# BindsNET/bindsnet

Measured on AMD Instinct MI355X. Metric: simulated timesteps/sec (whole node), DiehlAndCook2015 784->400 batch32, higher is better.
Workload: dtype f32

## Files before the change

### bindsnet_amd/_lib.py

```python
import ctypes as C
import os

_HERE = os.path.dirname(os.path.abspath(__file__))
LIB_PATH = os.path.join(_HERE, "lib", "libsnnhip.so")
if os.environ.get("SNN_DEVELOPER") == "1" and os.environ.get("SNN_LIB_OVERRIDE"):
    import warnings
    LIB_PATH = os.environ["SNN_LIB_OVERRIDE"]
    warnings.warn(f"bindsnet_amd: SNN_LIB_OVERRIDE is active, loading {LIB_PATH} instead of the in-tree library", RuntimeWarning)

SNN_OK, SNN_ERR_NOISE, SNN_ERR_TIMEOUT, SNN_ERR_RETRY = 0, -4, -6, -7
ABI_VERSION = 8


_EPOCH = [0]


def epoch() -> int:
    return _EPOCH[0]


def touch() -> None:
    _EPOCH[0] += 1


# ... 111 lines not shown
    "snn_dc_arbitrate": ([_vp, _vp, _i, _i, C.POINTER(DcParams), _vp, _ll, _vp, _vp, _vp, _vp], _i),
    "snn_stdp_postpre": ([_vp] * 5 + [_i, _i, _i, _f, _f, _i, _f, _f, _i, _f, _i, _f, _i, _vp], _i),
    "snn_conv2d_postpre": ([_vp] * 5 + [_i] * 9 + [_f, _f, _f, _i, _f, _i, _f, _vp, _vp], _i),
    "snn_stdp_hebbian": ([_vp] * 5 + [_i, _i, _i, _f, _f, _i, _f, _i, _f, _i, _f, _vp], _i),
    "snn_conv2d_mstdp_step": ([_vp] * 6 + [_i] * 8 + [_f] * 7 + [_i, _f, _i, _f, _vp], _i),
    "snn_mstdpet_step": ([_vp] * 8 + [_i, _i] + [_f] * 10 + [_i, _f, _i, _f, _vp], _i),
    "snn_mstdp_step": ([_vp] * 7 + [_i, _i, _i, _f, _vp, _f, _f, _f, _f, _f, _f, _i, _f, _i, _f, _vp], _i),
    "snn_normalize": ([_vp, _i, _i, _f, _i, _vp, _vp], _i),
    "snn_normalize_conv2d": ([_vp, _i, _i, _f, _vp], _i),
    "snn_rng_fill_exponential": ([_vp, _vp, _i, _i, _vp, _vp, _vp], _i),
    "snn_encode_bernoulli": ([_vp, _vp, _i, _i, _f, _vp, _vp], _i),
    "snn_encode_poisson": ([_vp, _i, _i, _f, C.c_ulonglong, _vp, _vp], _i),
    "snn_fill_segments": ([C.POINTER(FillSegment), _i, _vp], _i),
    "snn_dist_unique_id": ([_vp], _i),
    "snn_dist_init": ([_i, _i, _vp, C.POINTER(_vp)], _i),
    "snn_dist_world": ([_vp, C.POINTER(_i), C.POINTER(_i)], _i),
    "snn_dist_allreduce_dw": ([_vp, _vp, _ll, _vp], _i),
    "snn_dist_allgather_step": ([_vp, _vp, _vp, _ll, _vp], _i),
    "snn_dist_destroy": ([_vp], _i),
    "snn_net_run": ([C.POINTER(LayerDesc), _i, C.POINTER(ConnDesc), _i, C.POINTER(RunDesc), _vp], _i),
    "snn_net_workspace_bytes": ([C.POINTER(LayerDesc), _i, C.POINTER(ConnDesc), _i, C.POINTER(RunDesc)], C.c_ulonglong),
    "snn_plan_name": ([], C.c_char_p),
    "snn_dc2015_last_form": ([], C.c_int),
    "snn_set_plan_mode": ([_i], None),
    "snn_graph_stats": ([C.POINTER(C.c_int)] * 3, None),
    "snn_profile_enable": ([_i], None),
    "snn_profile_collect": ([C.POINTER(C.c_double), C.POINTER(C.c_int)], _i),
}


def exported_symbols():
    return sorted(_SIGS)


def lib():
    global _lib
    if _lib is None:
        if not os.path.exists(LIB_PATH):
            raise SnnError(f"{LIB_PATH} is missing: build it with `make -C bindsnet_amd/csrc` "
                           "(python __graft_entry__.py build). There is no fallback path.")
        L = C.CDLL(LIB_PATH)
        for name, (args, res) in _SIGS.items():
            fn = getattr(L, name)
            fn.argtypes, fn.restype = args, res
        if L.snn_abi_version() != ABI_VERSION:
            raise SnnError(f"libsnnhip ABI {L.snn_abi_version()} != binding {ABI_VERSION}")
# ... 33 lines not shown
        try:
            for _ in range(max(1, repeats)):
                net.run(dict(inputs), time=time)
                net.reset_state_variables()
                if not net.last_plan.startswith("dc2015-resident"):
                    break
            net.sync()
            torch.cuda.synchronize()
            s, n = C.c_double(0), C.c_int(0)
            check(L.snn_profile_collect(C.byref(s), C.byref(n)), "profile_collect")
        finally:
            L.snn_profile_enable(0)
    if n.value == 0:
        return None
    plan = net.last_plan
    if plan.startswith("dc2015-resident"):
        form = L.snn_dc2015_last_form()
        return {"kernel": resident_kernel_name(form) + " (one launch per network.run())", "resident_form": form, "avg_ms": s.value / n.value, "n": n.value,
                "timesteps_per_launch": int(round(time / net.dt))}
    kernel = "k_dc2015_step (one launch per timestep)" if plan != "generic" else "generic plan: all launches of one timestep"
    return {"kernel": kernel, "avg_ms": s.value / n.value, "n": n.value, "timesteps_per_launch": 1}


def graph_stats():
    a, b, c = C.c_int(0), C.c_int(0), C.c_int(0)
    lib().snn_graph_stats(C.byref(a), C.byref(b), C.byref(c))
    return a.value, b.value, c.value
```

### bindsnet_amd/csrc/snn_dc2015.hip

```cpp
#include <string.h>
#include <stdio.h>
#include <stdlib.h>
#include <vector>
#include <algorithm>
#include "snn_dc2015.hpp"

unsigned long long snn_twolayer_workspace_bytes(const snn_layer_desc *L, int nL, const snn_conn_desc *C, int nC,
                                                const snn_run_desc *R);
bool snn_prof_begin(int t, hipStream_t st);
bool snn_prof_active();
void snn_prof_end(hipStream_t st);

namespace {

template <class SUM, bool FULL>
__device__ __forceinline__ void stdp_rows(const DcCtx &c, int nact, const uint16_t *arows, const uint32_t *rowmask,
                                          const uint32_t *colmask, const uint8_t *__restrict__ sbytes,
                                          const float *xnu0, const float *__restrict__ xsrc, float *wtile, int c0, int tid,
                                          int Emain, const float *pre_w) {
    const int B = c.B, Nin = c.Nin, N = c.N;
    const int nitems = nact * CW;
    const int q = tid % CW;
    for (int base = 0; base < nitems; base += NT * 8) {
        float wv[8]; int ev[8]; int iv[8];
// ... 501 lines not shown
}

size_t lds_bytes(int B, int Nin, int N) {
    const int NW = (N + 31) / 32;
    auto al = [](size_t x) { return (x + 15) & ~(size_t)15; };
    return al((size_t)digest_lds_words(B, Nin) * 4) + 3 * al((size_t)B * NW * 4) +
           (size_t)MAXB * CW * 4 + 8 * 624 * 4 + NCAND * 4 + MAXB * 8 + 2 * MAXB * LR * 2 + 2 * MAXB * 4 + 2 * 32 * 4 + 32 +
           (size_t)Nin * CW * 4 + 2 * MAXB * CW * 4;
}


}

static size_t fused_workspace(int B, int Nin, int N) {
    const int NW = (N + 31) / 32;
    auto al = [](size_t x) { return (x + 255) & ~(size_t)255; };
    return 4 * al((size_t)B * NW * 4) + al((size_t)B * Nin * 4) + al(sizeof(snn_rng_state));
}

static thread_local int g_last_form = -1;
static thread_local unsigned long long g_ws_key_in = 0;
void snn_dc2015_ws_key_in(unsigned long long key) { g_ws_key_in = key; }
constexpr int kAsyncDefault = 1;
static size_t resident_summary_bytes(int N) { return (size_t)4 * ((N + 1) / 2) * 4 * 8; }
static size_t resident_gran_bytes(int B, int N) { return (size_t)4 * ((N + 1) / 2) * ((B + 1) / 2) * 8; }
constexpr size_t kAsyncCtlBytes = 8 * 11 * 8 + 16 * 4 + 64;

static size_t resident_second_bytes(int B, int N) {
    auto al = [](size_t x) { return (x + 255) & ~(size_t)255; };
    return al(resident_gran_bytes(B, N)) + al(resident_summary_bytes(N));
}
static size_t resident_extra(int B, int Nin, int N, int T) {
    auto al = [](size_t x) { return (x + 255) & ~(size_t)255; };
    return al(resident_gran_bytes(B, N)) + al(resident_summary_bytes(N)) + al(kAsyncCtlBytes) + al((size_t)(T + 1 + 16) * 4) + al((size_t)(T + 1) * B * Nin * 4) +
           2 * resident_second_bytes(B, N);
}

constexpr size_t kResidentMaxExtra = (size_t)2 << 30;

static size_t fused_workspace_total(int B, int Nin, int N, int T) {
    auto al = [](size_t x) { return (x + 255) & ~(size_t)255; };
    const size_t extra = resident_extra(B, Nin, N, T);
    return fused_workspace(B, Nin, N) + al((size_t)(T + 1) * digest_words(B, Nin) * 4) + (extra <= kResidentMaxExtra ? extra : 0);
}

static bool matches(const snn_layer_desc *L, int nL, const snn_conn_desc *C, int nC, const snn_run_desc *R) {
    if (nL != 3 || nC != 3) return false;
    if (L[0].kind != SNN_LAYER_INPUT || L[1].kind != SNN_LAYER_DC || L[2].kind != SNN_LAYER_LIF) return false;
    if (L[1].n != L[2].n) return false;
    for (int k = 0; k < 3; ++k) if (C[k].kind != SNN_CONN_MCC || C[k].bias) return false;
    if (C[0].src != 0 || C[0].dst != 1 || C[1].src != 1 || C[1].dst != 2 || C[2].src != 2 || C[2].dst != 1) return false;
    if (C[1].rule != SNN_RULE_NONE || C[2].rule != SNN_RULE_NONE) return false;
    if (C[0].rule != SNN_RULE_NONE && C[0].rule != SNN_RULE_POSTPRE) return false;
    if (C[0].rule == SNN_RULE_POSTPRE && (C[0].wdecay != 1.0f || !L[0].x || !L[1].x)) return false;
    if (R->B > MAXB) return false;
    if (L[0].n > 2048 || L[0].n % 16 != 0 || L[1].n > 1024 || R->B * ((L[1].n + 31) / 32) > NT) return false;
    if ((size_t)R->B * L[0].n > (size_t)NU * NT * 16) return false;
    if ((double)(R->T + 1) * R->B * L[0].n >= 2147483648.0) return false;
    if (L[1].p.one_spike && !R->rng) return false;
    if (R->T < 1) return false;
    if (lds_bytes(R->B, L[0].n, L[1].n) > 150 * 1024) return false;
    if (!R->workspace || R->workspace_bytes < fused_workspace_total(R->B, L[0].n, L[1].n, R->T)) return false;
    if (digest_lds_words(R->B, L[0].n) > 4 * NT) return false;
    return true;
}

extern "C" int snn_dc2015_last_form(void) { return g_last_form; }

unsigned long long snn_twolayer_workspace_bytes(const snn_layer_desc *L, int nL, const snn_conn_desc *C, int nC, const snn_run_desc *R);
unsigned long long snn_convpp_workspace_bytes(const snn_layer_desc *L, int nL, const snn_conn_desc *C, int nC, const snn_run_desc *R);
extern "C" unsigned long long snn_net_workspace_bytes(const snn_layer_desc *L, int nL, const snn_conn_desc *C, int nC,
                                          const snn_run_desc *R) {
    if (!L || !R || !C) return 0;
    if (nL == 2 && nC == 1) {
        const unsigned long long w = snn_twolayer_workspace_bytes(L, nL, C, nC, R);
        return w ? w : snn_convpp_workspace_bytes(L, nL, C, nC, R);
    }
    if (nL != 3 || nC != 3) return 0;
    return fused_workspace_total(R->B, L[0].n, L[1].n, R->T);
}

void snn_set_plan_name(const char *name);
uint8_t *snn_input_raster_request(int layer);
void snn_input_raster_done(int layer);
unsigned long long snn_twolayer_workspace_bytes(const snn_layer_desc *L, int nL, const snn_conn_desc *C, int nC,
                                                const snn_run_desc *R);
int g_graph_stats[3] = {0, 0, 0};

extern "C" void snn_graph_stats(int *h_plain, int *h_captured, int *h_replayed) {
    if (h_plain) *h_plain = g_graph_stats[0];
// ... 63 lines not shown
        while (rcw < 8 && ((N + rcw - 1) / rcw > cap(rcw) || snn_dc2015_resident_lds(B, Nin, N, rcw) > 150 * 1024)) rcw *= 2;
        if ((N + rcw - 1) / rcw > cap(rcw)) resident = 0;
    }
    const int rG = (N + rcw - 1) / rcw, rKB = (B + 16 / rcw - 1) / (16 / rcw);
    if ((c.rule == SNN_RULE_POSTPRE && !c.x_traces) || snn_dc2015_resident_lds(B, Nin, N, rcw) > 150 * 1024 ||
        resident_extra(B, Nin, N, R->T) > kResidentMaxExtra) resident = 0;
    int rnt = rnt0;
    if (rnt == 512 && (rcw > 4 || B * c.NW > 512)) rnt = 1024;
    static const bool lean_on = !(getenv("SNN_DC_LEAN") && atoi(getenv("SNN_DC_LEAN")) == 0);
    const bool lean1 = resident && allow_lean && lean_on && rcw == 4 && rnt == 1024 && L[1].p.one_spike &&
                       ((size_t)Nin * N) % 32 == 0 && Nin <= 1024 && 1024 - MAXB * 4 >= B * 4 * 4;
    static const bool spec_on = !(getenv("SNN_DC_SPEC") && atoi(getenv("SNN_DC_SPEC")) == 0);
    int lean = !lean1 ? 0 : (spec_on && snn_dc2015_spec_lds(B, Nin, N) <= 150 * 1024 ? 2 : 1);
    {
        const int async_env = getenv("SNN_DC_ASYNC") ? atoi(getenv("SNN_DC_ASYNC")) : kAsyncDefault;
        if (lean && async_env && N <= 1024 && B <= MAXB) {
            const size_t alds = snn_dc2015_async_lds(B, Nin, N);
            const int nrw = (c.rasE || c.rasI) ? 4 : 0;
            const int cap3 = alds <= 150 * 1024 ? snn_dc2015_async_capacity(alds) : 0;
            if (alds <= 150 * 1024 && rG + 1 + nrw <= cap3) {
                lean = 3;
                c.NRW = nrw;
                c.tbad = (int *)((unsigned char *)c.rprog + 16 * 4);
                const char *pe = getenv("SNN_DC_PRODUCERS");
                const int spare = cap3 - (rG + 1 + nrw), want = pe ? atoi(pe) : 128;
                c.NP = (want > 0 && spare >= 16 && dc_prep_lds_bytes(B, Nin, 512) <= alds) ? (spare < want ? spare : want) : 0;
                uint8_t *rq = c.NP > 0 ? snn_input_raster_request(0) : nullptr;
                if (rq && !(((uintptr_t)rq | (uintptr_t)c.in) & 15)) c.rasX = rq;
            }
        }
    }
    if (resident) { c.G = rG; c.KB = rKB; }
    static long long *dbg = nullptr;
    static int dbg_T = 0;
    if (getenv("SNN_DC_TIMING")) {
        const size_t dbg_words = (size_t)(24 + 256 * 4) * (R->T + 1);
        if (!dbg || dbg_T < R->T + 1) { if (dbg) (void)hipFree(dbg); (void)hipMalloc(&dbg, sizeof(long long) * dbg_words); dbg_T = R->T + 1; }
        (void)hipMemsetAsync(dbg, 0, sizeof(long long) * dbg_words, st);
        for (int t = 0; t <= R->T; ++t) (void)hipMemsetAsync(dbg + (size_t)t * 24 + 20, 0x7F, sizeof(long long), st);
        c.dbg = dbg; c.dbg_wg = atoi(getenv("SNN_DC_TIMING")); if (c.dbg_wg != -1 && (c.dbg_wg < 0 || c.dbg_wg >= c.G)) c.dbg_wg = c.G - 1;
    }
    const size_t lds = lds_bytes(B, Nin, N);
    static bool lds_attr = false;
    if (!lds_attr) {
        if (snn_check(hipFuncSetAttribute((const void *)k_dc2015_step, hipFuncAttributeMaxDynamicSharedMemorySize, 150 * 1024))) return SNN_ERR_LAUNCH;
        lds_attr = true;
// ... 13 lines not shown
            };
            unsigned long long key = 0x5EEDull;
            for (unsigned long long v : {(unsigned long long)(uintptr_t)c.ex, (unsigned long long)B, (unsigned long long)Nin, (unsigned long long)N, (unsigned long long)R->T,
                                         (unsigned long long)lean, (unsigned long long)exbytes, (unsigned long long)secbytes})
                key = mix(key, v);
            key |= 1ull;
            const bool clean = chain && g_ws_key_in == key;
            if (!clean) {
                if ((rc0 = snn_check(hipMemsetAsync(c.ex, 0, exbytes, qs)))) return rc0;
                if (chain && (rc0 = snn_check(hipMemsetAsync(sec0, 0, 2 * secbytes, qs)))) return rc0;
            }
            if (!(lean == 3 && c.NP > 0)) {
                hipLaunchKernelGGL(k_dc2015_prep, dim3(R->T + 1), dim3(NT), dc_prep_lds_bytes(B, Nin, NT), qs, c);
                if (c.x_traces) hipLaunchKernelGGL(k_dc2015_xtrace, dim3((B * Nin + 255) / 256), dim3(256), 0, qs, c);
            }
            const bool prof = with_events && snn_prof_begin(0, qs);
            static const bool section_coop = getenv("SNN_DC_SECTION_COOP") && atoi(getenv("SNN_DC_SECTION_COOP")) != 0;
            const bool ordinary = chain && !section_coop;
            int rcl = lean == 3 ? snn_dc2015_async_launch(c, snn_dc2015_async_lds(B, Nin, N), qs, ordinary)
                                : snn_dc2015_resident_launch(c, rcw, rnt, lean == 2 ? snn_dc2015_spec_lds(B, Nin, N) : snn_dc2015_resident_lds(B, Nin, N, rcw), lean, qs);
            if (prof) snn_prof_end(qs);
            if (rcl == SNN_OK && lean && R->status2) {
                DcCtx c2 = c;
                c2.tbad = nullptr; c2.NRW = 0; c2.NP = 0; c2.rasX = nullptr; c2.status = R->status2; c2.gate = R->status;
                if (chain) {
                    const int par = (int)(R->host_state[1] & 1ull);
                    unsigned char *mine = sec0 + (size_t)par * secbytes, *other = sec0 + (size_t)(par ^ 1) * secbytes;
                    c2.ex = (unsigned long long *)mine;
                    c2.exs = (unsigned long long *)(mine + al(resident_gran_bytes(B, N)));
                    c2.zeroA = (uint4 *)c.ex; c2.zeroA_n16 = (unsigned)(exbytes >> 4);
                    c2.zeroG = (uint4 *)other; c2.zeroG_n16 = (unsigned)(secbytes >> 4);
                } else if ((rc0 = snn_check(hipMemsetAsync(c.ex, 0, exbytes, qs)))) return rc0;
                static const bool gated_coop = getenv("SNN_DC_GATED_COOP") && atoi(getenv("SNN_DC_GATED_COOP")) != 0;
                rcl = snn_dc2015_resident_launch(c2, rcw, rnt, snn_dc2015_resident_lds(B, Nin, N, rcw), 0, qs, !gated_coop && !section_coop);
                if (rcl == SNN_OK && chain) { R->host_state[0] = key; R->host_state[1] += 1; }
            }
            if (rcl == SNN_OK && lean == 3 && c.rasX) snn_input_raster_done(0);
            return rcl;
        }
        rc0 = snn_check(hipMemsetAsync(ws, 0, 4 * wb, qs));
        if (rc0) return rc0;
        hipLaunchKernelGGL(k_dc2015_prep, dim3(R->T + 1), dim3(NT), dc_prep_lds_bytes(B, Nin, NT), qs, c);
        for (int t = 0; t <= R->T; ++t) {
            const bool prof = with_events && snn_prof_begin(t, qs);
            hipLaunchKernelGGL(k_dc2015_step, dim3(c.G), dim3(NT), lds, qs, c, t);
            if (prof) snn_prof_end(qs);
        }
// ... 229 lines not shown
```

### bindsnet_amd/csrc/snn_dc2015.hpp

```cpp
#pragma once
#include <hip/hip_runtime.h>
#include <stdint.h>
#include "../../include/snnhip.h"
#include "snn_common.hpp"
#include "snn_order.hpp"
#include "snn_rng.hpp"

struct DcCtx {
    int B, Nin, N, T, NW, NinW, G, RS;
    float dt; int learning;
    const uint8_t *in;
    const uint8_t *sX0;
    float *xX[2];
    int x_traces; float x_decay, x_scale; int x_additive;
    float *vE, *rE, *xE, *theta; uint8_t *sE;
    snn_dc_params pE;
    uint8_t *rasE; float *rasVE;
    float *vI, *rI, *xI; uint8_t *sI;
    snn_lif_params pI;
    uint8_t *rasI; float *rasVI;
    float *Wxe; const float *Wei; const float *Wie;
    int rule; float nu0, nu1; int use_dt; int has_min; float wmin; int has_max; float wmax;
    uint32_t *crossE[2], *spikeI[2];
    snn_rng_state *rng[2];
    float inv_hwps, inv_NW, inv_RS;
    uint32_t *dig; int DW, DGW, OXW;
    unsigned long long *ex; int KB;
    unsigned long long *exs;
    float *xtr;
    int *status;
    int has_norm; float norm; int norm_abs;
    int zone_shift;
    int spec_flags;
    int rows4;
    int stall_wg;
    int dbg_wg;
    long long *dbg;
    unsigned long long *wing;
    int *rprog;
    int NRW;
    int *tbad;
    const int *gate;
    int *dready;
    int NP;
    uint8_t *rasX;
    uint4 *zeroA, *zeroG;
    unsigned zeroA_n16, zeroG_n16;
};

namespace {
using namespace snn;

constexpr int CW = 8;
constexpr int MAXB = 32;
constexpr int TT = MAXB * CW;
constexpr int NT = 1024;
constexpr int NU = 2;

__device__ __forceinline__ void lds_barrier() { asm volatile("s_waitcnt lgkmcnt(0)\n\ts_barrier" ::: "memory"); }


#define DBG_MARK(slot) do { if (c.dbg && blockIdx.x == c.dbg_wg && threadIdx.x == 0) c.dbg[(size_t)t * 24 + (slot)] = (long long)wall_clock64(); } while (0)

__device__ __forceinline__ bool bit_of(const uint32_t *w, int j) { return (w[j >> 5] >> (j & 31)) & 1u; }

__device__ __forceinline__ uint32_t nz4(uint32_t w) {
    const uint32_t t = (w | ((w & 0x7f7f7f7fu) + 0x7f7f7f7fu)) & 0x80808080u;
    return ((t >> 7) | (t >> 14) | (t >> 21) | (t >> 28)) & 0xFu;
}

template <class SUM>
// ... 290 lines not shown
```

### bindsnet_amd/csrc/snn_dc2015_async.hip

```cpp
#include <limits.h>
#include <stdlib.h>
#include "snn_dc2015.hpp"
#include "snn_dc2015_tile.hpp"

namespace {

constexpr int ACW = 4;
constexpr int ANT = 512;
constexpr int kCrossRing = 4;
constexpr int kWinRing = 8;
constexpr int kWinGr = 11;
constexpr int kArbRing = 32;
constexpr unsigned kAPoll = 400000u;
constexpr unsigned kAbortPay = 0xFFFFFFFEu;

__device__ __forceinline__ uint32_t win_tag(int e) { return (uint32_t)(e + 1) & 1023u; }

__device__ __forceinline__ void report(int *status, int code) {
    if (status) atomicCAS(status, 0, code);
}

__device__ __forceinline__ const DcCtx &cold(const DcCtx &) {
    const __attribute__((address_space(4))) DcCtx *p = (const __attribute__((address_space(4))) DcCtx *)__builtin_amdgcn_kernarg_segment_ptr();
    asm volatile("" : "+s"(p));
    return *(const DcCtx *)p;
}

constexpr int AT = MAXB * ACW;
constexpr size_t OC_CTL = 0, OC_XNU0 = 128, OC_XNU0S = OC_XNU0 + 2 * AT * 4, OC_CURX = OC_XNU0S + AT * 4, OC_CURXW = OC_CURX + 2 * AT * 4,
                 OC_SPFIN = OC_CURXW + AT * 4, OC_THC = OC_SPFIN + AT * 4, OC_COLM = OC_THC + 32, OC_COLX = OC_COLM + 32, OC_COLRES = OC_COLX + 32,
                 OC_XWINV = OC_COLRES + 16, OC_XCNT = OC_XWINV + 16 + 16, OC_W0 = OC_XCNT + 2 * MAXB * 4, OC_C0 = OC_W0 + 2 * MAXB * 4, OC_WT = OC_C0 + 2 * MAXB * 4;
static_assert(OC_WT % 16 == 0 && OC_XNU0 % 16 == 0 && OC_XNU0S % 16 == 0, "16-byte aligned float4 arrays");
size_t async_compute_lds(int B, int Nin, int N) {
    const int DGS = (digest_lds_words(B, Nin) + 63) & ~63;
    return OC_WT + (size_t)3 * Nin * ACW * 4 + (size_t)2 * N * ACW * 4 + (size_t)2 * DGS * 4;
}
constexpr size_t OA_CTL = 0, OA_CNT = 128, OA_COL = 256, OA_WL = 384, OA_KEY = 512, OA_CRS = 1280;
size_t async_arbiter_lds(int B, int N) {
    const int BW = (B * ((N + 31) / 32) + 3) & ~3;
    return OA_CRS + (size_t)BW * 4 + (size_t)kArbRing * 624 * 4;
}

template <bool DUAL>
__device__ __forceinline__ float x_current4(const float *ws, const float *ws2, float &out2, const uint32_t *dg, int B, int Nin, int pb, int pq,
                                            int pL, bool tailcol) {
    constexpr int CW = ACW;
    constexpr uint32_t GM = (1u << GCB) - 1u;
    const uint16_t *lstX = (const uint16_t *)dg;
    const uint32_t *rowmask = dg + B * (LX / 2) + 40;
    const uint16_t *arows = (const uint16_t *)(rowmask + Nin);
    const uint16_t *lst2 = arows + 4 * ((Nin + 1) / 2);
    const uint32_t *gcnt = (const uint32_t *)(lst2 + B * LX);
    const uint32_t *gqn = gcnt + B;
    if (tailcol) {
// ... 200 lines not shown
#pragma unroll
        for (int k = 0; k < 4; ++k) if (k < GL) A2 = A2 + Gs[k];
        float Gl = 0.0f;
#pragma unroll
        for (int k = 0; k < 4; ++k) if (k == GL) Gl = Gs[k];
        const float res = ((0.0f + Gl) + A2) + 0.0f;
        r[q] = 0.0f + res;
    }
    return make_float4(r[0], r[1], r[2], r[3]);
}

__device__ __forceinline__ void scan_entry(const DcCtx &c, int *w0, int *cnt0, int tid) {
    const int B = c.B, N = c.N;
    if (tid < 2 * MAXB) { w0[tid] = -1; cnt0[tid] = 0; }
    __syncthreads();
    for (int k = tid; k < B * N; k += ANT) {
        if (c.sE[k]) { const int b = k / N; atomicAdd(&cnt0[b], 1); w0[b] = k - b * N; }
        if (c.sI[k]) { const int b = k / N; atomicAdd(&cnt0[MAXB + b], 1); w0[MAXB + b] = k - b * N; }
    }
    __syncthreads();
}

constexpr int kWinPollSleep = 1;
struct WinPre { unsigned long long g0; bool have; };
__device__ __forceinline__ WinPre win_prefetch(const DcCtx &c, int e, int myb) {
    WinPre p; p.g0 = granule_load(c.wing + (size_t)(e & (kWinRing - 1)) * kWinGr + myb / 3); p.have = true;
    return p;
}
__device__ __forceinline__ int sample_winner(const DcCtx &c, const int *w0, int e, int myb, bool &bad, WinPre pre = WinPre{0ull, false}) {
    if (e < 0) return w0[(e == -1 ? 0 : MAXB) + myb];
    const unsigned long long *gr = c.wing + (size_t)(e & (kWinRing - 1)) * kWinGr + myb / 3;
    const uint32_t tag = win_tag(e);
    unsigned long long x0 = pre.have ? pre.g0 : granule_load(gr);
    for (unsigned spins = 0; __any((uint32_t)(x0 >> 54) != tag); ++spins) {
        if (spins > kAPoll) { bad = true; report(cold(c).status, SNN_ERR_TIMEOUT); return -1; }
        __builtin_amdgcn_s_sleep(kWinPollSleep);
        x0 = granule_load(gr);
    }
    if (__any((int)((x0 >> 48) & 63u) == 63)) { bad = true; return -1; }
    const uint32_t w = (uint32_t)(x0 >> (16 * (myb % 3))) & 0xFFFFu;
    return w == 0xFFFFu ? -1 : (int)(w & 0x7FFu);
}

#define AMARKW(k, th) do { if constexpr (TIMING) { if (c.dbg && g == c.dbg_wg && tid == (th)) c.dbg[(size_t)t * 24 + (k)] = (long long)wall_clock64(); } } while (0)
#define AMARK(k) do { if constexpr (TIMING) { if (wave == 0 && c.dbg_wg >= 0) mk[k] = (long long)wall_clock64(); } } while (0)
#define AMARK2(k) do { if constexpr (TIMING) { if (wave == 2 && c.dbg_wg >= 0) mk[k] = (long long)wall_clock64(); } } while (0)
#define AMARK2_FLUSH() do { if constexpr (TIMING) { if (c.dbg && g == c.dbg_wg && tid == 128 && t >= 1) { _Pragma("unroll") for (int k_ = 19; k_ < 24; ++k_) c.dbg[(size_t)(t - 1) * 24 + k_] = mk[k_]; } } } while (0)
#define AMARK_FLUSH() do { if constexpr (TIMING) { if (c.dbg && g == c.dbg_wg && tid == 0) { _Pragma("unroll") for (int k_ = 0; k_ < 19; ++k_) { \
        const bool early_ = k_ == 0 || k_ == 9 || k_ == 10 || k_ == 7 || k_ == 11 || k_ == 18; \
        if (k_ != 3 && k_ != 17 && (early_ || t >= 1)) c.dbg[(size_t)(early_ ? t : t - 1) * 24 + k_] = mk[k_]; } } } } while (0)

__device__ __forceinline__ float vgpr(float x) { float r; asm volatile("v_mov_b32 %0, %1" : "=v"(r) : "s"(x)); return r; }
__device__ __forceinline__ snn_lif_params vgpr_params(snn_lif_params p) {
    p.decay = vgpr(p.decay); p.rest = vgpr(p.rest); p.reset = vgpr(p.reset); p.thresh = vgpr(p.thresh); p.refrac = vgpr(p.refrac);
    p.dt = vgpr(p.dt); p.lbound = vgpr(p.lbound); p.trace_decay = vgpr(p.trace_decay); p.trace_scale = vgpr(p.trace_scale);
    return p;
// ... 128 lines not shown
        __builtin_amdgcn_s_sleep(4);
    }
    __builtin_amdgcn_fence(__ATOMIC_ACQUIRE, "agent");
    all = true;
    return 1;
}

template <bool TIMING, bool FT>
__device__ __forceinline__ void async_compute(const DcCtx &c, unsigned char *smem) {
    constexpr int CW = ACW, TT = AT, NT = ANT, NTW = TT / 64, SPW = 64 / CW, SPG = 16 / CW, NBC = NT - TT, TI0 = NT - TT;
    const int B = FT ? MAXB : c.B, Nin = c.Nin, N = c.N, T = c.T;
    int *ctl = (int *)(smem + OC_CTL);
    float *xnu0 = (float *)(smem + OC_XNU0);
    float *xnu0s = (float *)(smem + OC_XNU0S);
    float *curX = (float *)(smem + OC_CURX);
    float *curXwin = (float *)(smem + OC_CURXW);
    int *spfin = (int *)(smem + OC_SPFIN);
    int *thc = (int *)(smem + OC_THC);
    uint32_t *colmask = (uint32_t *)(smem + OC_COLM);
    uint32_t *colx = (uint32_t *)(smem + OC_COLX);
    uint32_t *colres = (uint32_t *)(smem + OC_COLRES);
    float *xwinv = (float *)(smem + OC_XWINV);
    int *xcnt = (int *)(smem + OC_XCNT);
    int *w0 = (int *)(smem + OC_W0), *cnt0 = (int *)(smem + OC_C0);
    float *wtile = (float *)(smem + OC_WT);
    float *wieT = wtile + (size_t)Nin * CW;
    float *weiT = wieT + (size_t)N * CW;
    const int DGS = (c.DGW + 63) & ~63;
    uint32_t *dgbuf = (uint32_t *)(weiT + (size_t)N * CW);
    float *wbak = (float *)(dgbuf + 2 * DGS);
    float *wwin = wbak + (size_t)Nin * CW;

    const int tid = threadIdx.x, lane = tid & 63, wave = tid >> 6;
    const int g = (int)blockIdx.x, c0 = g * CW;
    const bool is_ai = tid >= TI0;
    const int ptile = is_ai ? tid - TI0 : tid;
    const int jj = ptile % CW, bl = ptile / CW, j = c0 + jj;
    const bool colv = FT ? true : j < N, tailcol = c0 >= (N / 32) * 32;
    const bool mine = FT ? tid < TT : (tid < TT && bl < B && colv);
    const bool mine_i = FT ? is_ai : (is_ai && bl < B && colv);
    const unsigned kst = (unsigned)(bl * N + j);
    const int NGS = c.G * NTW;
    const snn_lif_params pE = vgpr_params(c.pE.lif), pI = vgpr_params(c.pI);
    const float theta_plus = vgpr(c.pE.theta_plus), theta_decay = vgpr(c.pE.theta_decay);
    const PPar pp = {vgpr(c.nu0), vgpr(c.nu1), vgpr(c.dt), vgpr(c.wmin), vgpr(c.wmax), c.use_dt, c.has_min, c.has_max};
    const bool e_learning = c.pE.learning != 0;
// ... 56 lines not shown
    }
    if (tid < TT) {
        float xn = 0.f;
        if (bl < B && colv && pE.traces) xn = trace_next(x_cur, 0, pE.trace_decay, pE.trace_scale, pE.traces_additive);
        xnu0[tid] = xn * pp.nu0; xnu0[TT + tid] = 0.f; xnu0s[tid] = 0.f;
        curX[tid] = 0.f; curX[TT + tid] = 0.f; curXwin[tid] = 0.f;
        spfin[tid] = (mine && last_s) ? 1 : 0;
    }
    asm volatile("s_waitcnt vmcnt(0)" ::: "memory");
    __syncthreads();
    bool bad = ctl[0] != 0;
    if (bad && tid == 0) report(c.status, SNN_ERR_RETRY);
    for (int qt = tid; qt < B * CW * 4; qt += NT) {
        const int pb = qt / (CW * 4), pq = (qt >> 2) % CW, pL = qt & 3;
        float unused = 0.f;
        const float v = x_current4<false>(wtile, wtile, unused, dgbuf, B, Nin, pb, pq, pL, tailcol);
        if (pL == 0 && c0 + pq < N) curX[pb * CW + pq] = v;
    }
    lds_barrier();
    bool sp_prev = false;
    bool crossed_prev = false;
    unsigned long long prevE = 0ull;
    int published = 0;
    WinPre pre_w = WinPre{0ull, false};
    const bool learn_pp = c.learning && c.rule == SNN_RULE_POSTPRE;

    if constexpr (TIMING) {
        if (c.dbg && tid == 0) {
            c.dbg[(size_t)24 * (T + 1) + ((size_t)T * 256 + g) * 4 + 2] = (long long)(__builtin_amdgcn_s_getreg((31 << 11) | 20) & 0xF);
            c.dbg[(size_t)24 * (T + 1) + ((size_t)T * 256 + g) * 4 + 3] = (long long)(__builtin_amdgcn_s_getreg((31 << 11) | 4) & 0xFFFFFF);
        }
    }
    long long mk[24] = {0, 0, 0, 0, 0, 0, 0, 0, 0, 0, 0, 0, 0, 0, 0, 0, 0, 0, 0, 0, 0, 0, 0, 0};
    (void)mk;
    bool prev_anyx = true;
    auto step_loop = [&](auto role_c) __attribute__((always_inline)) {
    constexpr int ROLE = decltype(role_c)::value;
    constexpr bool R_TILE = ROLE == 0, R_F4 = ROLE == 1, R_W4 = ROLE == 2, R_AI = ROLE == 3, R_NT = ROLE != 0;
    (void)R_W4; (void)R_AI; (void)R_F4;
    for (int t = 0; t <= T; ++t) {
        const bool phaseB = t < T;
        const int par = t & 1;
        const uint32_t *dgn = dgbuf + (par ^ 1) * DGS;
        const int *meta = (const int *)(dgn + B * (LX / 2));
        const uint32_t *rowmask = dgn + B * (LX / 2) + 40;
        const uint16_t *arows = (const uint16_t *)(rowmask + Nin);
        const bool do_stdp = phaseB && learn_pp;
        const bool full = t == 0;
        AMARK(0);
        AMARK2_FLUSH();
        if constexpr (TIMING) { if (c.dbg && tid == 0 && c.dbg_wg >= 0) c.dbg[(size_t)24 * (T + 1) + ((size_t)t * 256 + g) * 4 + 0] = (long long)wall_clock64(); }
        if (t + 2 <= T && R_NT) {
            if (PENDING(1)) {
                bool all = false;
                const int r = need_entry(cold(c), t + 2, all);
                if (r != 1) { ctl[0] = 1; report(cold(c).status, r < 0 ? SNN_ERR_TIMEOUT : SNN_ERR_RETRY); }
                if (all) pend &= ~1;
            }
            DIGEST_LOAD_E(t + 2);
        }
        float cx_plain = 0.f;
        int thc_prev = 0;
// ... 3 lines not shown
        uint32_t wonm = 0;
        if (learn_pp && prev_anyx) {
#pragma unroll
            for (int q = 0; q < CW; ++q) wonm |= (__builtin_amdgcn_readfirstlane((int)colmask[par * CW + q]) != 0 ? 1u : 0u) << q;
        }
        AMARK(10);
        if (!phaseB) {
            if (wonm)
                for (int i = tid; i < Nin; i += NT) {
                    float4 v = *(const float4 *)(wtile + i * 4);
                    const float4 ww = *(const float4 *)(wwin + i * 4);
                    if (wonm & 1u) v.x = ww.x;
                    if (wonm & 2u) v.y = ww.y;
                    if (wonm & 4u) v.z = ww.z;
                    if (wonm & 8u) v.w = ww.w;
                    *(float4 *)(wtile + i * 4) = v;
                }
            break;
        }
        if (R_TILE) {

            float cx = 0.f;
            if (mine) cx = ((wonm >> jj) & 1u) ? curXwin[bl * CW + jj] : cx_plain;
            if constexpr (TIMING) { if (c.dbg && g == c.dbg_wg && tid == 0) c.dbg[(size_t)t * 24 + 17] = !pre_w.have ? 2 : ((uint32_t)(pre_w.g0 >> 54) != win_tag(t - 2) ? 1 : 0); }
            const int jI = bad ? -1 : sample_winner(c, w0, t - 2, min(bl, B - 1), bad, pre_w);
            AMARK(7);
            AMARK_FLUSH();
            bool spE = false;
            if (mine) {
                const float e2 = jI >= 0 ? wieT[min(jI, N - 1) * CW + jj] * 1.0f + 0.0f : 0.0f;
                const float curE = cx + e2;
                if (e_learning && t >= 1) r_th = r_th + theta_plus * (float)thc_prev;
                if (e_learning) r_th = r_th * theta_decay;
                spE = dc_update(r_v, r_r, curE, pE.thresh + r_th, pE);
                if (spE) atomicAdd(&thc[par * CW + jj], 1);
            }
            const uint64_t mE = __ballot(spE);
            AMARK(12);
            const int slot = t & (kCrossRing - 1);
            uint32_t pay;
            if (bad) pay = kAbortPay;
            else {
                const int nev = __popcll(mE);
                if (nev <= 3) {
                    pay = (uint32_t)nev << 30;
                    int sh = 0;
                    for (uint64_t m = mE; m; m &= m - 1) { pay |= (uint32_t)(__ffsll((unsigned long long)m) - 1) << sh; sh += 8; }
                } else {
                    const int sidx = lane / CW, b = wave * SPW + sidx;
                    const uint32_t v = (uint32_t)((mE >> (sidx * CW)) & 0xFFFFull);
// ... 63 lines not shown
                *(float4 *)(wbak + i * 4) = v;
                *(float4 *)(wtile + i * 4) = postpre_row_nowin(pp, v, m, xn0);
            }
            if (wonm && !full)
                for (int i = ptid; i < Nin; i += NBC) {
                    if (rowmask[i] != 0) continue;
                    float4 v = *(const float4 *)(wtile + i * 4);
                    const float4 ww = *(const float4 *)(wwin + i * 4);
                    if (wonm & 1u) v.x = ww.x;
                    if (wonm & 2u) v.y = ww.y;
                    if (wonm & 4u) v.z = ww.z;
                    if (wonm & 8u) v.w = ww.w;
                    *(float4 *)(wtile + i * 4) = v;
                }
            AMARKW(3, TT);
        }
        if (t + 2 <= T && R_NT) DIGEST_STORE_E(t + 2);
        AMARK(13);
        lds_barrier();
        AMARK(4);

        if constexpr (TIMING) { if (c.dbg && tid == 0 && c.dbg_wg >= 0) c.dbg[(size_t)24 * (T + 1) + ((size_t)t * 256 + g) * 4 + 3] = (long long)wall_clock64(); }
        if (tid < CW) { colmask[par * CW + tid] = 0; colx[(par ^ 1) * CW + tid] = 0; thc[(par ^ 1) * CW + tid] = 0; }
        if (R_TILE) { pre_w.have = false; if (t >= 1 && t + 1 < T) pre_w = win_prefetch(c, t - 1, min(bl, B - 1)); }
        constexpr bool f4w = R_F4;
        if (f4w) {
            const int ptid = tid - TT, pb = ptid >> 2, pL = ptid & 3;
            const float4 v = x_current_f4(wtile, dgn, B, Nin, min(pb, B - 1), pL, tailcol);
            if (pL == 0 && pb < B) *(float4 *)(curX + (par ^ 1) * TT + pb * CW) = v;
        }
        uint32_t xq[CW];
#pragma unroll
        for (int q = 0; q < CW; ++q) xq[q] = (uint32_t)__builtin_amdgcn_readfirstlane((int)colx[par * CW + q]);
        const bool crossed_wg = do_stdp && (xq[0] | xq[1] | xq[2] | xq[3]) != 0u;
        prev_anyx = (xq[0] | xq[1] | xq[2] | xq[3]) != 0u;
        if (crossed_wg && PENDING(2)) {
            bool all = false;
            if (need_xtr(cold(c), all) != 1) { ctl[0] = 1; report(cold(c).status, SNN_ERR_TIMEOUT); }
            if (all) pend &= ~2;
        }
        const float *xsrc = crossed_wg ? cold(c).xtr + (size_t)(t + 1) * B * Nin : nullptr;
        const float *xn0 = xnu0 + par * TT;
        uint32_t cmq[CW];
#pragma unroll
        for (int q = 0; q < CW; ++q) cmq[q] = crossed_wg ? xq[q] : 0u;
        const int nact = !phaseB ? 0 : (full ? Nin : __builtin_amdgcn_readfirstlane(meta[32]));
        AMARK(14);
// ... 135 lines not shown
        AMARK(2);
    }
    };
    if (wave < NTW) step_loop(std::integral_constant<int, 0>{});
    else if (wave < NTW + 2) step_loop(std::integral_constant<int, 1>{});
    else if (wave < NTW + 4) step_loop(std::integral_constant<int, 2>{});
    else step_loop(std::integral_constant<int, 3>{});
    if (PENDING(2) && !bad) {
        bool all = false;
        if (need_xtr(cold(c), all) != 1) { bad = true; report(cold(c).status, SNN_ERR_TIMEOUT); }
    }
    if (wave < NTW && lane == 0) {
        const int pstep = (bad && published <= T - 1) ? published : T;
        granule_store(c.exs + (size_t)(pstep & (kCrossRing - 1)) * NGS + g * NTW + wave, ((unsigned long long)(uint32_t)(pstep + 1) << 32) | (bad ? kAbortPay : 0u));
    }
    asm volatile("s_waitcnt vmcnt(0)" ::: "memory");
    if (wave == 0 && !bad) {
        bool b2 = false;
        (void)sample_winner(c, w0, T, 0, b2);
        if (!b2 && lane == 0) ctl[1] = 1;
    }
    __syncthreads();
    if (ctl[0] != 0 || ctl[1] == 0) return;
    if (c.x_traces) {
        const float *src = c.xtr + (size_t)T * B * Nin;
        for (int k = g * NT + tid; k < B * Nin; k += c.G * NT) c.xX[1][k] = src[k];
    }
    if (mine) {
        float th = r_th;
        if (e_learning) th = th + theta_plus * (float)thc[((T - 1) & 1) * CW + jj];
        c.vE[kst] = r_v; c.rE[kst] = r_r;
        if (bl == 0) c.theta[j] = th;
        if (pE.traces) c.xE[kst] = x_cur;
        c.sE[kst] = last_s;
    }
    if (mine_i) {
        c.vI[kst] = r_v; c.rI[kst] = r_r;
        if (pI.traces) c.xI[kst] = x_cur;
        c.sI[kst] = last_s;
    }
    if (c.has_norm) {
        float *bsum = (float *)dgbuf;
        float *sc = xnu0;
        const int nfull = Nin >> 4;
        __syncthreads();
        if (!tailcol) {
// ... 416 lines not shown
```

### include/snnhip.h

```cpp
#ifndef SNNHIP_H
#define SNNHIP_H

#include <stdint.h>

#ifdef __cplusplus
extern "C" {
#endif

#define SNN_ABI_VERSION 8

typedef void *snn_stream_t;

enum {
    SNN_OK = 0,
    SNN_ERR_INVALID = -1,
    SNN_ERR_UNSUPPORTED = -2,
    SNN_ERR_LAUNCH = -3,
    SNN_ERR_NOISE = -4,
    SNN_ERR_NO_DEVICE = -5,
    SNN_ERR_TIMEOUT = -6,
    SNN_ERR_RETRY = -7
};

int snn_abi_version(void);
// ... 186 lines not shown
    int B, T;
    float dt;
    int learning;
    const float *noise_q;
    long long q_len;
    snn_rng_state *rng;
    float *qbuf;
    void *workspace;
    unsigned long long workspace_bytes;
    long long *cursor;
    int *status;
    int one_step;
    int plan;
    int *status2;
    unsigned long long *host_state;
} snn_run_desc;

int snn_net_run(const snn_layer_desc *h_layers, int n_layers, const snn_conn_desc *h_conns, int n_conns,
                const snn_run_desc *h_run, snn_stream_t stream);
unsigned long long snn_net_workspace_bytes(const snn_layer_desc *h_layers, int n_layers, const snn_conn_desc *h_conns,
                                           int n_conns, const snn_run_desc *h_run);
const char *snn_plan_name(void);
int snn_dc2015_last_form(void);
void snn_profile_enable(int stride);
int snn_profile_collect(double *h_sum_ms, int *h_samples);
void snn_graph_stats(int *h_plain, int *h_captured, int *h_replayed);
void snn_set_plan_mode(int mode);

typedef struct snn_dist snn_dist;
int snn_dist_unique_id(void *h_id128);
int snn_dist_init(int rank, int world, const void *h_id128, snn_dist **h_out);
int snn_dist_world(const snn_dist *d, int *h_rank, int *h_world);
int snn_dist_allreduce_dw(snn_dist *d, float *buf, long long count, snn_stream_t stream);
int snn_dist_allgather_step(snn_dist *d, const void *send, void *recv, long long bytes_per_rank, snn_stream_t stream);
int snn_dist_destroy(snn_dist *d);

#ifdef __cplusplus
}
#endif
#endif
```

Before: 293,700.

## Resolve inhibitory winner directly from exchange granules, lag arbiter check

Each workgroup now reads the per-wave spike summary granules from the cross ring and works out the winner itself when at most one excitatory neuron fired per batch row. It falls back to waiting on the arbiter's winner ring only when there are ties. The arbiter ring is still checked, but kArbLag steps behind, for abort detection, and the cross ring is widened from 4 to 8 entries so it can hold that lag. This takes the arbiter round-trip off the per-step critical path. The cost is more granule loads, LDS atomics, a larger workspace, and new counters plus an API for how many steps took the direct versus arbiter path.

```diff
diff --git a/bindsnet_amd/_lib.py b/bindsnet_amd/_lib.py
--- a/bindsnet_amd/_lib.py
+++ b/bindsnet_amd/_lib.py
@@ -157,6 +157,7 @@
     "snn_net_workspace_bytes": ([C.POINTER(LayerDesc), _i, C.POINTER(ConnDesc), _i, C.POINTER(RunDesc)], C.c_ulonglong),
     "snn_plan_name": ([], C.c_char_p),
     "snn_dc2015_last_form": ([], C.c_int),
+    "snn_dc2015_winner_paths": ([C.POINTER(C.c_int)] * 2, _i),
     "snn_set_plan_mode": ([_i], None),
     "snn_graph_stats": ([C.POINTER(C.c_int)] * 3, None),
     "snn_profile_enable": ([_i], None),
@@ -236,6 +237,12 @@
     return {"kernel": kernel, "avg_ms": s.value / n.value, "n": n.value, "timesteps_per_launch": 1}
 
 
+def dc2015_winner_paths():
+    a, b = C.c_int(0), C.c_int(0)
+    check(lib().snn_dc2015_winner_paths(C.byref(a), C.byref(b)), "dc2015_winner_paths")
+    return a.value, b.value
+
+
 def graph_stats():
     a, b, c = C.c_int(0), C.c_int(0), C.c_int(0)
     lib().snn_graph_stats(C.byref(a), C.byref(b), C.byref(c))
diff --git a/bindsnet_amd/csrc/snn_dc2015.hip b/bindsnet_amd/csrc/snn_dc2015.hip
--- a/bindsnet_amd/csrc/snn_dc2015.hip
+++ b/bindsnet_amd/csrc/snn_dc2015.hip
@@ -547,8 +547,14 @@
 static thread_local unsigned long long g_ws_key_in = 0;
 void snn_dc2015_ws_key_in(unsigned long long key) { g_ws_key_in = key; }
 constexpr int kAsyncDefault = 1;
-static size_t resident_summary_bytes(int N) { return (size_t)4 * ((N + 1) / 2) * 4 * 8; }
-static size_t resident_gran_bytes(int B, int N) { return (size_t)4 * ((N + 1) / 2) * ((B + 1) / 2) * 8; }
+static size_t resident_summary_bytes(int N) {
+    const size_t a = (size_t)4 * ((N + 1) / 2) * 4 * 8, b = (size_t)kAsyncCrossRing * ((N + 3) / 4) * 2 * 8;
+    return a > b ? a : b;
+}
+static size_t resident_gran_bytes(int B, int N) {
+    const size_t a = (size_t)4 * ((N + 1) / 2) * ((B + 1) / 2) * 8, b = (size_t)kAsyncCrossRing * ((N + 3) / 4) * ((B + 3) / 4) * 8;
+    return a > b ? a : b;
+}
 constexpr size_t kAsyncCtlBytes = 8 * 11 * 8 + 16 * 4 + 64;
 
 static size_t resident_second_bytes(int B, int N) {
@@ -591,6 +597,27 @@
 }
 
 extern "C" int snn_dc2015_last_form(void) { return g_last_form; }
+
+static int *winner_paths_words() {
+    static int *words[16] = {nullptr};
+    int dev = 0;
+    if (hipGetDevice(&dev) != hipSuccess || dev < 0 || dev >= 16) { (void)hipGetLastError(); return nullptr; }
+    if (!words[dev]) {
+        int *p = nullptr;
+        if (hipMalloc(&p, 2 * sizeof(int)) != hipSuccess || hipMemset(p, 0, 2 * sizeof(int)) != hipSuccess) { (void)hipGetLastError(); return nullptr; }
+        words[dev] = p;
+    }
+    return words[dev];
+}
+extern "C" int snn_dc2015_winner_paths(int *h_direct_steps, int *h_arbiter_steps) {
+    int h[2] = {0, 0};
+    int *w = winner_paths_words();
+    if (!w) return SNN_ERR_LAUNCH;
+    if (int rc = snn_check(hipMemcpy(h, w, sizeof(h), hipMemcpyDeviceToHost))) return rc;
+    if (h_direct_steps) *h_direct_steps = h[0];
+    if (h_arbiter_steps) *h_arbiter_steps = h[1];
+    return SNN_OK;
+}
 
 unsigned long long snn_twolayer_workspace_bytes(const snn_layer_desc *L, int nL, const snn_conn_desc *C, int nC, const snn_run_desc *R);
 unsigned long long snn_convpp_workspace_bytes(const snn_layer_desc *L, int nL, const snn_conn_desc *C, int nC, const snn_run_desc *R);
@@ -700,6 +727,7 @@
                 lean = 3;
                 c.NRW = nrw;
                 c.tbad = (int *)((unsigned char *)c.rprog + 16 * 4);
+                c.wpaths = winner_paths_words();
                 const char *pe = getenv("SNN_DC_PRODUCERS");
                 const int spare = cap3 - (rG + 1 + nrw), want = pe ? atoi(pe) : 128;
                 c.NP = (want > 0 && spare >= 16 && dc_prep_lds_bytes(B, Nin, 512) <= alds) ? (spare < want ? spare : want) : 0;
@@ -759,7 +787,7 @@
             if (prof) snn_prof_end(qs);
             if (rcl == SNN_OK && lean && R->status2) {
                 DcCtx c2 = c;
-                c2.tbad = nullptr; c2.NRW = 0; c2.NP = 0; c2.rasX = nullptr; c2.status = R->status2; c2.gate = R->status;
+                c2.tbad = nullptr; c2.NRW = 0; c2.NP = 0; c2.rasX = nullptr; c2.wpaths = nullptr; c2.status = R->status2; c2.gate = R->status;
                 if (chain) {
                     const int par = (int)(R->host_state[1] & 1ull);
                     unsigned char *mine = sec0 + (size_t)par * secbytes, *other = sec0 + (size_t)(par ^ 1) * secbytes;
diff --git a/bindsnet_amd/csrc/snn_dc2015.hpp b/bindsnet_amd/csrc/snn_dc2015.hpp
--- a/bindsnet_amd/csrc/snn_dc2015.hpp
+++ b/bindsnet_amd/csrc/snn_dc2015.hpp
@@ -46,7 +46,10 @@
     uint8_t *rasX;
     uint4 *zeroA, *zeroG;
     unsigned zeroA_n16, zeroG_n16;
+    int *wpaths;
 };
+
+constexpr int kAsyncCrossRing = 8;
 
 namespace {
 using namespace snn;
diff --git a/bindsnet_amd/csrc/snn_dc2015_async.hip b/bindsnet_amd/csrc/snn_dc2015_async.hip
--- a/bindsnet_amd/csrc/snn_dc2015_async.hip
+++ b/bindsnet_amd/csrc/snn_dc2015_async.hip
@@ -7,8 +7,10 @@
 
 constexpr int ACW = 4;
 constexpr int ANT = 512;
-constexpr int kCrossRing = 4;
+constexpr int kCrossRing = kAsyncCrossRing;
+constexpr int kArbLag = 6;
 constexpr int kWinRing = 8;
+static_assert((kCrossRing & (kCrossRing - 1)) == 0 && kArbLag >= 2 && kArbLag < kCrossRing && kArbLag <= kWinRing - 2, "ring argument");
 constexpr int kWinGr = 11;
 constexpr int kArbRing = 32;
 constexpr unsigned kAPoll = 400000u;
@@ -29,7 +31,7 @@
 constexpr int AT = MAXB * ACW;
 constexpr size_t OC_CTL = 0, OC_XNU0 = 128, OC_XNU0S = OC_XNU0 + 2 * AT * 4, OC_CURX = OC_XNU0S + AT * 4, OC_CURXW = OC_CURX + 2 * AT * 4,
                  OC_SPFIN = OC_CURXW + AT * 4, OC_THC = OC_SPFIN + AT * 4, OC_COLM = OC_THC + 32, OC_COLX = OC_COLM + 32, OC_COLRES = OC_COLX + 32,
-                 OC_XWINV = OC_COLRES + 16, OC_XCNT = OC_XWINV + 16 + 16, OC_W0 = OC_XCNT + 2 * MAXB * 4, OC_C0 = OC_W0 + 2 * MAXB * 4, OC_WT = OC_C0 + 2 * MAXB * 4;
+                 OC_XWINV = OC_COLRES + 16, OC_XCNT = OC_XWINV + 16 + 16, OC_XCOL = OC_XCNT + 2 * MAXB * 4, OC_W0 = OC_XCOL + 2 * MAXB * 4, OC_C0 = OC_W0 + 2 * MAXB * 4, OC_WT = OC_C0 + 2 * MAXB * 4;
 static_assert(OC_WT % 16 == 0 && OC_XNU0 % 16 == 0 && OC_XNU0S % 16 == 0, "16-byte aligned float4 arrays");
 size_t async_compute_lds(int B, int Nin, int N) {
     const int DGS = (digest_lds_words(B, Nin) + 63) & ~63;
@@ -276,16 +278,11 @@
 }
 
 constexpr int kWinPollSleep = 1;
-struct WinPre { unsigned long long g0; bool have; };
-__device__ __forceinline__ WinPre win_prefetch(const DcCtx &c, int e, int myb) {
-    WinPre p; p.g0 = granule_load(c.wing + (size_t)(e & (kWinRing - 1)) * kWinGr + myb / 3); p.have = true;
-    return p;
-}
-__device__ __forceinline__ int sample_winner(const DcCtx &c, const int *w0, int e, int myb, bool &bad, WinPre pre = WinPre{0ull, false}) {
+__device__ __forceinline__ int sample_winner(const DcCtx &c, const int *w0, int e, int myb, bool &bad) {
     if (e < 0) return w0[(e == -1 ? 0 : MAXB) + myb];
     const unsigned long long *gr = c.wing + (size_t)(e & (kWinRing - 1)) * kWinGr + myb / 3;
     const uint32_t tag = win_tag(e);
-    unsigned long long x0 = pre.have ? pre.g0 : granule_load(gr);
+    unsigned long long x0 = granule_load(gr);
     for (unsigned spins = 0; __any((uint32_t)(x0 >> 54) != tag); ++spins) {
         if (spins > kAPoll) { bad = true; report(cold(c).status, SNN_ERR_TIMEOUT); return -1; }
         __builtin_amdgcn_s_sleep(kWinPollSleep);
@@ -460,6 +457,7 @@
     uint32_t *colres = (uint32_t *)(smem + OC_COLRES);
     float *xwinv = (float *)(smem + OC_XWINV);
     int *xcnt = (int *)(smem + OC_XCNT);
+    int *xcol = (int *)(smem + OC_XCOL);
     int *w0 = (int *)(smem + OC_W0), *cnt0 = (int *)(smem + OC_C0);
     float *wtile = (float *)(smem + OC_WT);
     float *wieT = wtile + (size_t)Nin * CW;
@@ -562,7 +560,7 @@
     bool crossed_prev = false;
     unsigned long long prevE = 0ull;
     int published = 0;
-    WinPre pre_w = WinPre{0ull, false};
+    int n_direct = 0, n_arb = 0;
     const bool learn_pp = c.learning && c.rule == SNN_RULE_POSTPRE;
 
     if constexpr (TIMING) {
@@ -578,6 +576,8 @@
     constexpr int ROLE = decltype(role_c)::value;
     constexpr bool R_TILE = ROLE == 0, R_F4 = ROLE == 1, R_W4 = ROLE == 2, R_AI = ROLE == 3, R_NT = ROLE != 0;
     (void)R_W4; (void)R_AI; (void)R_F4;
+    constexpr int PGX = 8;
+    unsigned long long xg[PGX] = {0ull, 0ull, 0ull, 0ull, 0ull, 0ull, 0ull, 0ull}, ag = 0ull;
     for (int t = 0; t <= T; ++t) {
         const bool phaseB = t < T;
         const int par = t & 1;
@@ -627,10 +627,81 @@
 
             float cx = 0.f;
             if (mine) cx = ((wonm >> jj) & 1u) ? curXwin[bl * CW + jj] : cx_plain;
-            if constexpr (TIMING) { if (c.dbg && g == c.dbg_wg && tid == 0) c.dbg[(size_t)t * 24 + 17] = !pre_w.have ? 2 : ((uint32_t)(pre_w.g0 >> 54) != win_tag(t - 2) ? 1 : 0); }
-            const int jI = bad ? -1 : sample_winner(c, w0, t - 2, min(bl, B - 1), bad, pre_w);
+            int jI = -1;
+            if (t < 2) {
+                if constexpr (TIMING) { if (c.dbg && g == c.dbg_wg && tid == 0) c.dbg[(size_t)t * 24 + 17] = 2; }
+                if (!bad) jI = sample_winner(c, w0, t - 2, min(bl, B - 1), bad);
+            } else if (!bad) {
+                const unsigned long long *sums = c.exs + (size_t)((t - 2) & (kCrossRing - 1)) * NGS;
+                const uint32_t xtag = (uint32_t)(t - 1);
+                uint32_t need = 0;
+#pragma unroll
+                for (int u = 0; u < PGX; ++u)
+                    if (64 * u < NGS && lane + 64 * u < NGS && (uint32_t)(xg[u] >> 32) != xtag) need |= 1u << u;
+                bool stale = __any(need != 0u);
+                if constexpr (TIMING) { if (c.dbg && g == c.dbg_wg && tid == 0) c.dbg[(size_t)t * 24 + 17] = stale ? 1 : 0; }
+                for (unsigned spins = 0; stale; ++spins) {
+                    if (spins > kAPoll) { bad = true; report(cold(c).status, SNN_ERR_TIMEOUT); break; }
+                    if (spins) __builtin_amdgcn_s_sleep(kWinPollSleep);
+#pragma unroll
+                    for (int u = 0; u < PGX; ++u) if (64 * u < NGS && ((need >> u) & 1u)) xg[u] = granule_load(sums + lane + 64 * u);
+#pragma unroll
+                    for (int u = 0; u < PGX; ++u) if (64 * u < NGS && ((need >> u) & 1u) && (uint32_t)(xg[u] >> 32) == xtag) need &= ~(1u << u);
+                    stale = __any(need != 0u);
+                }
+                AMARK(11);
+                uint32_t pv[PGX], anyp = 0;
+#pragma unroll
+                for (int u = 0; u < PGX; ++u) { pv[u] = (64 * u < NGS && lane + 64 * u < NGS) ? (uint32_t)xg[u] : 0u; anyp |= pv[u]; }
+                if (bad) {
+                } else if (!__any(anyp != 0u)) {
+                    ++n_direct;
+                } else {
+                    int *xc = xcnt + wave * MAXB, *xo = xcol + wave * MAXB;
+                    if (lane < MAXB) xc[lane] = 0;
+                    bool ab = false;
+#pragma unroll
+                    for (int u = 0; u < PGX; ++u) {
+                        const uint32_t pay = pv[u];
+                        if (!pay) continue;
+                        if (pay == kAbortPay) { ab = true; continue; }
+                        const int gi = lane + 64 * u, gsrc = gi / NTW, w = gi % NTW;
+                        if ((pay & 0xFFu) == 0xFFu) {
+                            for (int bs = 0; bs < SPW; ++bs) atomicAdd(&xc[w * SPW + bs], 2);
+                        } else {
+                            const int ne = (int)(pay >> 30);
+                            for (int e2 = 0; e2 < ne; ++e2) {
+                                const int p_ = (int)((pay >> (8 * e2)) & 0x3Fu), bsm = w * SPW + p_ / CW;
+                                atomicAdd(&xc[bsm], 1);
+                                xo[bsm] = gsrc * CW + p_ % CW;
+                            }
+                        }
+                    }
+                    asm volatile("s_waitcnt lgkmcnt(0)" ::: "memory");
+                    if (__any(ab)) bad = true;
+                    else {
+                        const int cnt = xc[bl];
+                        jI = cnt == 1 ? xo[bl] : -1;
+                        if (__any(cnt > 1)) {
+                            const int ja = sample_winner(c, w0, t - 2, min(bl, B - 1), bad);
+                            if (cnt > 1) jI = ja;
+                            ++n_arb;
+                        } else ++n_direct;
+                    }
+                }
+            }
             AMARK(7);
             AMARK_FLUSH();
+            if (t >= kArbLag && !bad) {
+                const unsigned long long *pa = c.wing + (size_t)((t - kArbLag) & (kWinRing - 1)) * kWinGr;
+                const uint32_t atag = win_tag(t - kArbLag);
+                for (unsigned spins = 0; __any((uint32_t)(ag >> 54) != atag); ++spins) {
+                    if (spins > kAPoll) { bad = true; report(cold(c).status, SNN_ERR_TIMEOUT); break; }
+                    __builtin_amdgcn_s_sleep(kWinPollSleep);
+                    ag = granule_load(pa);
+                }
+                if (!bad && __any((int)((ag >> 48) & 63u) == 63)) bad = true;
+            }
             bool spE = false;
             if (mine) {
                 const float e2 = jI >= 0 ? wieT[min(jI, N - 1) * CW + jj] * 1.0f + 0.0f : 0.0f;
@@ -740,7 +811,12 @@
 
         if constexpr (TIMING) { if (c.dbg && tid == 0 && c.dbg_wg >= 0) c.dbg[(size_t)24 * (T + 1) + ((size_t)t * 256 + g) * 4 + 3] = (long long)wall_clock64(); }
         if (tid < CW) { colmask[par * CW + tid] = 0; colx[(par ^ 1) * CW + tid] = 0; thc[(par ^ 1) * CW + tid] = 0; }
-        if (R_TILE) { pre_w.have = false; if (t >= 1 && t + 1 < T) pre_w = win_prefetch(c, t - 1, min(bl, B - 1)); }
+        if (R_TILE && t >= 1 && t + 1 < T) {
+            const unsigned long long *sums = c.exs + (size_t)((t - 1) & (kCrossRing - 1)) * NGS;
+#pragma unroll
+            for (int u = 0; u < PGX; ++u) if (64 * u < NGS && lane + 64 * u < NGS) xg[u] = granule_load(sums + lane + 64 * u);
+            if (t + 1 >= kArbLag) ag = granule_load(c.wing + (size_t)((t + 1 - kArbLag) & (kWinRing - 1)) * kWinGr);
+        }
         constexpr bool f4w = R_F4;
         if (f4w) {
             const int ptid = tid - TT, pb = ptid >> 2, pL = ptid & 3;
@@ -922,6 +998,7 @@
     }
     __syncthreads();
     if (ctl[0] != 0 || ctl[1] == 0) return;
+    if (g == 0 && tid == 0 && c.wpaths) { c.wpaths[0] = n_direct; c.wpaths[1] = n_arb; }
     if (c.x_traces) {
         const float *src = c.xtr + (size_t)T * B * Nin;
         for (int k = g * NT + tid; k < B * Nin; k += c.G * NT) c.xX[1][k] = src[k];
diff --git a/include/snnhip.h b/include/snnhip.h
--- a/include/snnhip.h
+++ b/include/snnhip.h
@@ -232,6 +232,7 @@
                                            int n_conns, const snn_run_desc *h_run);
 const char *snn_plan_name(void);
 int snn_dc2015_last_form(void);
+int snn_dc2015_winner_paths(int *h_direct_steps, int *h_arbiter_steps);
 void snn_profile_enable(int stride);
 int snn_profile_collect(double *h_sum_ms, int *h_samples);
 void snn_graph_stats(int *h_plain, int *h_captured, int *h_replayed);
```

New measurement: 226,000. 23.1% lower.
